# schmrlng/MotionPlanning.jl

Measured on AMD Instinct MI355X. Metric: edges checked/sec + r-disc queries/sec, FMT* N=1e6 R^6, 1/2/4/8 MI355X, higher is better.
Workload: dtype f64

## Files before the change

motionplanning.jl_amd/csrc/kernels_order.hip:

```cpp
#include "mpfmt_internal.h"
#include <algorithm>

#define ORD_ID(k) ((k) & 0x03ffffffu)
#define ORD_COL(k) (((k) >> 26) & 15u)
#define ORD_THREADS 512
#define ORD_WAVES 8
#define ORD_COLS 16
#define ORD_NB 128
#define ORD_STG 2560
#define ORD_PRE 5
#define ORD_WAVES_EU 8
static_assert(ORD_STG >= MPFMT_ORD_MAXDEG, "a column the host lets through must fit the staging area");
static_assert(ORD_COLS * ORD_NB == ORD_THREADS * 4, "the segmented scan gives every thread four buckets");
static_assert(ORD_PRE * ORD_THREADS >= ORD_STG && ORD_STG % 32 == 0 && ORD_STG < 65536, "the prefetched records cover what the staging area holds; positions fit 16 bits");

struct ord_hdr {
    int32_t k[ORD_COLS];
    int32_t cb[ORD_COLS + 4];
    long long out[ORD_COLS];
    int32_t ho[ORD_COLS];
    int32_t n, pad_[3];
};
struct ord_shared {
    uint32_t cnt[ORD_COLS][ORD_NB / 2];
    uint32_t cur[ORD_COLS][ORD_NB / 2];
    ord_hdr h[2];
    int32_t g1, pcount, nextk, pad_;
    uint32_t bits[ORD_STG / 32];
};

__device__ __forceinline__ void lds_barrier()
{
    asm volatile("s_waitcnt lgkmcnt(0)\n\ts_barrier" ::: "memory");
}

struct ord_args {
    const uint32_t* qkey;
    const double* qd2;
    long long qcap;
    const int32_t* qlen;
    const int64_t* degs;
    int64_t tile_begin, tile_end;
    const int64_t* colptr;
    const int32_t* perm;
    const int32_t* iperm;
    int32_t* rowval;
    double* nzval;
    int32_t* rowpos;
    uint32_t bucket_mul;
    const int32_t* spec_fail;
    unsigned long long* mask;
    const int64_t* nnz_dev;
    uint4* pend_items; int64_t pend_wcap; int32_t* pend_cnt; int32_t* pend_over;
    int64_t* deg_clear;
    int rec_bits;
    int32_t* qctr;
};

__global__ __launch_bounds__(ORD_THREADS) __attribute__((amdgpu_waves_per_eu(ORD_WAVES_EU, ORD_WAVES_EU))) void k_order_logs(ord_args a)
{
    if (a.spec_fail && *a.spec_fail) return;
    extern __shared__ __attribute__((aligned(16))) char ord_smem[];
    double* const stage_d2 = reinterpret_cast<double*>(ord_smem);
    uint32_t* const stage_key = reinterpret_cast<uint32_t*>(ord_smem + ORD_STG * 8);
    ord_shared& sh = *reinterpret_cast<ord_shared*>(ord_smem + ORD_STG * 12);
    const int tid = threadIdx.x, lane = tid & 63;
    const int wave = __builtin_amdgcn_readfirstlane(tid >> 6);
    const int64_t nq = (a.tile_end - a.tile_begin) * 4;
    auto bucket = [&](uint32_t id) -> int { return a.bucket_mul ? min(ORD_NB - 1, (int)__umulhi(id, a.bucket_mul)) : (int)(id & (ORD_NB - 1)); };
    if (a.rec_bits && blockIdx.x == 0 && tid == 0) {
        const int64_t nnz = *a.nnz_dev;
        if (nnz & 63) atomicAnd(&a.mask[nnz >> 6], (1ull << (nnz & 63)) - 1ull);
    }

    int hk = 0, ho = -1, hln = 0;
    long long hout = 0;
    auto hdr_fetch1 = [&](int64_t qi) {
        hk = 0; ho = -1; hln = 0;
        if (qi >= nq) return;
        if (tid < ORD_COLS) {
            const int64_t sp = a.tile_begin * 64 + qi * ORD_COLS + tid;
            ho = a.perm[sp];
            hk = (int)a.degs[sp];
            if (a.deg_clear && ho >= 0) a.deg_clear[ho] = 0;
        } else if (tid == 64) {
            hln = (int)min((long long)a.qlen[qi], a.qcap);
        }
    };
    auto hdr_fetch2 = [&]() { hout = (tid < ORD_COLS && ho >= 0) ? a.colptr[ho] : 0; };
    auto hdr_publish = [&](int hb) {
        ord_hdr& H = sh.h[hb];
        if (tid < 64) {
            const int k = (tid < ORD_COLS && ho >= 0) ? hk : 0;
            int inc = k;
            inc += __builtin_amdgcn_update_dpp(0, inc, 0x111, 0xf, 0xf, true);
            inc += __builtin_amdgcn_update_dpp(0, inc, 0x112, 0xf, 0xf, true);
            inc += __builtin_amdgcn_update_dpp(0, inc, 0x114, 0xf, 0xf, true);
            inc += __builtin_amdgcn_update_dpp(0, inc, 0x118, 0xf, 0xf, true);
            if (tid < ORD_COLS) { H.k[tid] = k; H.cb[tid + 1] = inc; H.ho[tid] = ho; }
            if (tid == 0) H.cb[0] = 0;
        } else if (tid == 64) {
            H.n = hln;
        }
    };
    uint32_t pk[ORD_PRE];
    double pd[ORD_PRE];
    auto rec_fetch_n = [&](int total, int64_t qi) {
        const __amdgpu_buffer_rsrc_t rk = __builtin_amdgcn_make_buffer_rsrc(const_cast<uint32_t*>(a.qkey + (qi < nq ? qi : 0) * a.qcap), 0, total * 4, 0x00020000);
#pragma unroll
        for (int u = 0; u < ORD_PRE; ++u) pk[u] = __builtin_amdgcn_raw_buffer_load_b32(rk, tid * 4, u * ORD_THREADS * 4, 0);
    };
    auto rec_fetch = [&](const ord_hdr& H, int64_t qi) { rec_fetch_n((qi < nq) ? H.n : 0, qi); };
    typedef uint32_t ord_u32x2 __attribute__((ext_vector_type(2)));
    auto d2_fetch = [&](int total, int64_t qi) {
        const long long base = (qi < nq ? qi : 0) * a.qcap;
        const __amdgpu_buffer_rsrc_t rd = __builtin_amdgcn_make_buffer_rsrc(const_cast<double*>(a.qd2 + base), 0, total * 8, 0x00020000);
#pragma unroll
        for (int u = 0; u < ORD_PRE; ++u) {
            const ord_u32x2 v = __builtin_amdgcn_raw_buffer_load_b64(rd, tid * 8, u * ORD_THREADS * 8, 0);
            pd[u] = __hiloint2double((int)v.y, (int)v.x);
        }
    };

    if (tid == 0) sh.pcount = 0;
    int64_t qi = blockIdx.x;
    int64_t qn = qi + gridDim.x;
    const int xcd = (int)(blockIdx.x & 7u);
    int hb = 0;
    hdr_fetch1(qi);
    hdr_fetch2();
    hdr_publish(0);
    if (tid < ORD_COLS) sh.h[0].out[tid] = hout;
    lds_barrier();
    rec_fetch(sh.h[0], qi);
    d2_fetch(sh.h[0].n, qi);
    for (; qi < nq; hb ^= 1) {
        const ord_hdr& H = sh.h[hb];
        const int total = H.n;
        const long long lbase = qi * a.qcap;
        hdr_fetch1(qn);
            int g0 = 0;
        bool first = true;
        while (g0 < ORD_COLS) {
            if (tid < 64) {
                const bool ok = tid >= g0 && tid < ORD_COLS && (H.cb[min(tid, ORD_COLS - 1) + 1] - H.cb[g0] <= ORD_STG);
                const unsigned long long m = __ballot(ok);
                if (tid == 0) sh.g1 = g0 + (int)__popcll(m);
            }
            *reinterpret_cast<uint2*>(&sh.cnt[0][tid * 2]) = make_uint2(0u, 0u);
            lds_barrier();
            int g1 = sh.g1;
            const bool skip = g1 == g0;
            if (skip) g1 = g0 + 1;
            const int gb = H.cb[g0];
            auto for_records = [&](auto&& f) {
                if (first) {
#pragma unroll
                    for (int u = 0; u < ORD_PRE; ++u) if (u * ORD_THREADS + tid < total) {
                        uint32_t key = pk[u];
                        asm volatile("" : "+v"(key));
                        f(key, u, u * ORD_THREADS + tid);
                    }
                }
                for (int i = (first ? ORD_PRE * ORD_THREADS : 0) + tid; i < total; i += ORD_THREADS) f(a.qkey[lbase + i], -1, i);
            };
            if (!skip) for_records([&](uint32_t key, int, int) {
                const int col = (int)ORD_COL(key);
                if (col >= g0 && col < g1) { const int bk = bucket(ORD_ID(key)); atomicAdd(&sh.cnt[col][bk >> 1], 1u << ((bk & 1) * 16)); }
            });
            lds_barrier();
            {
                const int col = tid >> 5;
                const uint2 cw = *reinterpret_cast<const uint2*>(&sh.cnt[0][tid * 2]);
                const int c0 = (int)(cw.x & 0xffffu), c1 = (int)(cw.x >> 16), c2 = (int)(cw.y & 0xffffu), c3 = (int)(cw.y >> 16);
                const int tot = c0 + c1 + c2 + c3;
                int inc = tot;
                inc += __builtin_amdgcn_update_dpp(0, inc, 0x111, 0xf, 0xf, true);
                inc += __builtin_amdgcn_update_dpp(0, inc, 0x112, 0xf, 0xf, true);
                inc += __builtin_amdgcn_update_dpp(0, inc, 0x114, 0xf, 0xf, true);
                inc += __builtin_amdgcn_update_dpp(0, inc, 0x118, 0xf, 0xf, true);
                inc += __builtin_amdgcn_update_dpp(0, inc, 0x142, 0xa, 0xf, false);
                const int b0 = min(max(H.cb[col] - gb + inc - tot, 0), ORD_STG);
                const int b1 = min(b0 + c0, ORD_STG), b2 = min(b1 + c1, ORD_STG), b3 = min(b2 + c2, ORD_STG);
                *reinterpret_cast<uint2*>(&sh.cur[0][tid * 2]) = make_uint2((uint32_t)b0 | ((uint32_t)b1 << 16), (uint32_t)b2 | ((uint32_t)b3 << 16));
            }
            lds_barrier();
            if (!skip) for_records([&](uint32_t key, int u, int i) {
                const int col = (int)ORD_COL(key);
                if (col >= g0 && col < g1) {
                    const int bk = bucket(ORD_ID(key));
                    const int pos = (int)((atomicAdd(&sh.cur[col][bk >> 1], 1u << ((bk & 1) * 16)) >> ((bk & 1) * 16)) & 0xffffu);
                    double d2 = 0.0;
                    if (u < 0) d2 = a.qd2[lbase + i];
#pragma unroll
                    for (int v = 0; v < ORD_PRE; ++v) if (u == v) d2 = pd[v];
                    if (pos >= 0 && pos < ORD_STG) { stage_key[pos] = key; stage_d2[pos] = d2; }
                }
            });
            if (a.rec_bits && tid < ORD_STG / 32) sh.bits[tid] = 0xffffffffu;
            lds_barrier();
            if (first) {
                hdr_fetch2();
                hdr_publish(hb ^ 1);
                if (a.qctr && tid == 0) sh.nextk = atomicAdd(&a.qctr[xcd], 1);
                first = false;
            }
            const bool last_range = g1 >= ORD_COLS;
            if (last_range) {
                lds_barrier();
                rec_fetch(sh.h[hb ^ 1], qn);
                d2_fetch(qn < nq ? sh.h[hb ^ 1].n : 0, qn);
            }
            if (!skip) {
                const int nst = min(H.cb[g1] - gb, ORD_STG);
                for (int p0 = 0; p0 < nst; p0 += ORD_THREADS) {
                    const int p = p0 + tid;
                    const bool act = p < nst;
                    if (p0 + wave * 64 >= nst) break;
                    const uint32_t key = act ? stage_key[p] : ((uint32_t)(g1 - 1) << 26);
                    const int col = (int)ORD_COL(key);
                    const uint32_t id = ORD_ID(key);
                    const int bk = bucket(id);
                    const int e = (int)((sh.cur[col][bk >> 1] >> ((bk & 1) * 16)) & 0xffffu), n = (int)((sh.cnt[col][bk >> 1] >> ((bk & 1) * 16)) & 0xffffu);
                    int rk = e - n;
                    if (act) {
                        const int b0 = e - n, bl = e - 1;
                        const uint32_t m0 = ORD_ID(stage_key[b0]), m1 = ORD_ID(stage_key[min(b0 + 1, bl)]), m2 = ORD_ID(stage_key[min(b0 + 2, bl)]),
                                       m3 = ORD_ID(stage_key[min(b0 + 3, bl)]);
                        rk += (int)(m0 < id) + (int)(n > 1 && m1 < id) + (int)(n > 2 && m2 < id) + (int)(n > 3 && m3 < id);
                        for (int m = b0 + 4; m < e; ++m) rk += (ORD_ID(stage_key[m]) < id) ? 1 : 0;
                    }
                    const int rel = rk - (H.cb[col] - gb);
                    const bool valid = act && rel >= 0 && rel < H.k[col];
                    const int64_t o = H.out[col] + rel;
                    int32_t rp = 0;
                    const bool pd_ = valid && a.pend_items && ((key >> 30) & 1u);
                    if ((valid && a.rowpos) || pd_) rp = a.iperm[id];
                    if (valid) {
                        a.rowval[o] = (int32_t)id;
                        a.nzval[o] = sqrt(stage_d2[p]);
                        if (a.rowpos) a.rowpos[o] = rp;
                    }
                    if (a.rec_bits && valid && (key >> 31)) atomicAnd(&sh.bits[rk >> 5], ~(1u << (rk & 31)));
                    if (a.pend_items) {
                        const unsigned long long pm = __ballot(pd_);
                        if (pm) {
                            int base = 0;
                            if (lane == 0) base = atomicAdd(&sh.pcount, (int)__popcll(pm));
                            base = __builtin_amdgcn_readfirstlane(base);
                            if (pd_) {
                                const int pos = base + (int)__builtin_amdgcn_mbcnt_hi((uint32_t)(pm >> 32), __builtin_amdgcn_mbcnt_lo((uint32_t)pm, 0u));
                                if (pos < a.pend_wcap)
                                    a.pend_items[(int64_t)blockIdx.x * a.pend_wcap + pos] =
                                        make_uint4((uint32_t)(uint64_t)o, (uint32_t)((uint64_t)o >> 32), (uint32_t)H.ho[col], (uint32_t)rp);
                            }
                        }
                    }
                }
            }
            lds_barrier();
            if (a.rec_bits) {
                if (!skip) for (int c = g0 + 2 * wave; c < min(g1, g0 + 2 * wave + 2); ++c) {
                    const int k = H.k[c];
                    if (k == 0) continue;
                    const int sb = H.cb[c] - gb;
                    const int64_t o = H.out[c];
                    const int64_t w0 = o >> 6;
                    const int nw = (int)(((o + k - 1) >> 6) - w0) + 1;
                    for (int i = lane; i < nw; i += 64) {
                        const int64_t wd = w0 + i;
                        const int64_t lo_bit = max(wd * 64, o), hi_bit = min(wd * 64 + 64, o + k);
                        const int nb = (int)(hi_bit - lo_bit);
                        const int src = sb + (int)(lo_bit - o);
                        const int wi = src >> 5, sh5 = src & 31;
                        const unsigned long long a0 = sh.bits[wi], a1 = sh.bits[min(wi + 1, ORD_STG / 32 - 1)], a2 = sh.bits[min(wi + 2, ORD_STG / 32 - 1)];
                        unsigned long long val = (a0 | (a1 << 32)) >> sh5;
                        if (sh5) val |= a2 << (64 - sh5);
                        const unsigned long long keep = (nb == 64) ? ~0ull : ((1ull << nb) - 1ull);
                        const int dsh = (int)(lo_bit & 63);
                        const unsigned long long rng = keep << dsh;
                        const unsigned long long w64 = ((val & keep) << dsh) | ~rng;
                        if (w64 != ~0ull) atomicAnd(&a.mask[wd], w64);
                    }
                }
                lds_barrier();
            }
            g0 = g1;
        }
        if (tid < ORD_COLS) sh.h[hb ^ 1].out[tid] = hout;
        qi = qn;
        qn = a.qctr ? 2 * (int64_t)gridDim.x + xcd + 8 * (int64_t)sh.nextk : qn + gridDim.x;
    }
    if (a.pend_items) {
        lds_barrier();
        if (tid == 0) {
            const int c = sh.pcount;
            a.pend_cnt[blockIdx.x] = (int32_t)min((int64_t)c, a.pend_wcap);
            if (c > a.pend_wcap) *a.pend_over = 1;
        }
    }
}

int32_t mpfmt_mask_preset(mpfmt_ctx* ctx, int64_t entries)
{
    int32_t rc;
    const int64_t words = (entries + 63) / 64;
    if ((rc = ctx->graph_free.ensure(ctx, sizeof(uint64_t) * (size_t)(words + 1)))) return rc;
    HIPCHK(ctx, hipMemsetAsync(ctx->graph_free, 0xFF, sizeof(uint64_t) * (size_t)std::max<int64_t>(words, 1), ctx->stream));
    ctx->mask_preset_words = words;
    return MPFMT_OK;
}

int32_t mpfmt_order_logs(mpfmt_ctx* ctx, const int32_t* spec_fail, int64_t mask_entries)
{
    const int64_t nt = ctx->tile_end - ctx->tile_begin;
    int32_t rc;
    ctx->rowpos_valid = false;
    const bool recbits = ctx->bits_in_records;
    const bool pend = ctx->broad_in_drain && !recbits;
    if (recbits) {
        const int64_t words = (std::max<int64_t>(ctx->nnz, mask_entries) + 63) / 64;
        const int64_t words_alloc = (std::max<int64_t>((int64_t)((double)ctx->nnz * 1.02) + 4096, mask_entries) + 63) / 64 + 1;
        if ((rc = ctx->graph_free.ensure(ctx, sizeof(uint64_t) * (size_t)words_alloc))) return rc;
        if (!(ctx->mask_preset_words == words && ctx->nnz > 0))
            HIPCHK(ctx, hipMemsetAsync(ctx->graph_free, ctx->nnz > 0 ? 0xFF : 0, sizeof(uint64_t) * (size_t)std::max<int64_t>(words, 1), ctx->stream));
    }
    ctx->mask_preset_words = -1;
    if (ctx->nnz == 0 || nt <= 0) { if ((rc = mpfmt_side_join(ctx))) return rc; if (recbits) { ctx->graph_swept = true; ctx->sweep_epoch += 1; ctx->sweep_in_order = true; } return MPFMT_OK; }
    const bool want_rowpos = !pend && !recbits;
    if (want_rowpos && (rc = ctx->rowpos.ensure(ctx, sizeof(int32_t) * (size_t)std::max<int64_t>(std::max(ctx->nnz, ctx->nnz_cap), 1)))) return rc;
    const size_t lds = (size_t)ORD_STG * 12 + sizeof(ord_shared);
    HIPCHK(ctx, hipFuncSetAttribute((const void*)k_order_logs, hipFuncAttributeMaxDynamicSharedMemorySize, (int)lds));
    if (ctx->ord_per_cu == 0) {
        int per_cu = 0;
        HIPCHK(ctx, hipOccupancyMaxActiveBlocksPerMultiprocessor(&per_cu, k_order_logs, ORD_THREADS, lds));
        ctx->ord_per_cu = std::max(1, std::min(per_cu, 4));
    }
    unsigned nb = (unsigned)std::min<int64_t>(nt * 4, (int64_t)ctx->num_cus * ctx->ord_per_cu);
    const bool draw = ctx->ord_draw && ctx->ord_ctr && nb >= 8 && (ctx->ord_draw > 1 || ctx->nnz >= (int64_t)1536 * nt * 4);
    if (draw) nb &= ~3u;
    if (pend) {
        const int64_t entries = std::max<int64_t>(ctx->nnz, ctx->nnz_cap);
        ctx->pend_wcap = ctx->debug_small_lists ? 8 : entries * 3 / (2 * (int64_t)nb) + 4096;
        if ((rc = ctx->pend_items.ensure(ctx, sizeof(uint4) * (size_t)ctx->pend_wcap * nb))) return rc;
        if ((rc = ctx->pend_cnt.ensure(ctx, sizeof(int32_t) * (size_t)(nb + 1)))) return rc;
        ctx->pend_over = ctx->pend_cnt + nb;
        HIPCHK(ctx, hipMemsetAsync(ctx->pend_over, 0, sizeof(int32_t), ctx->stream));
    }
    ord_args a{};
    a.qkey = ctx->qkey; a.qd2 = ctx->qd2; a.qcap = ctx->qcap; a.qlen = ctx->qlen; a.degs = ctx->degs;
    a.tile_begin = ctx->tile_begin; a.tile_end = ctx->tile_end; a.colptr = ctx->colptr; a.perm = ctx->perm; a.iperm = ctx->iperm;
    a.rowval = ctx->rowval; a.nzval = ctx->nzval; a.rowpos = want_rowpos ? ctx->rowpos : nullptr;
    a.bucket_mul = ctx->N > 128 ? (uint32_t)((128ull << 32) / (uint64_t)ctx->N) : 0u;
    a.spec_fail = spec_fail;
    a.mask = (unsigned long long*)ctx->graph_free.get(); a.nnz_dev = ctx->colptr + ctx->N;
    a.pend_items = pend ? (uint4*)ctx->pend_items.get() : nullptr; a.pend_wcap = ctx->pend_wcap; a.pend_cnt = ctx->pend_cnt; a.pend_over = ctx->pend_over;
    a.rec_bits = recbits ? 1 : 0;
    a.deg_clear = ctx->world > 1 ? ctx->deg : nullptr;
    a.qctr = draw ? ctx->ord_ctr : nullptr;
    if ((rc = mpfmt_side_join(ctx))) return rc;
    hipLaunchKernelGGL(k_order_logs, dim3(nb), dim3(ORD_THREADS), lds, ctx->stream, a);
    HIPCHK(ctx, hipGetLastError());
    if (pend) ctx->pend_nseg = (int)nb;
    ctx->pend_valid = pend;
    ctx->rowpos_valid = want_rowpos;
    if (recbits) { ctx->graph_swept = true; ctx->sweep_epoch += 1; ctx->sweep_in_order = true; }
    return MPFMT_OK;
}
```

motionplanning.jl_amd/csrc/mpfmt_internal.h:

```cpp
#pragma once
#include <hip/hip_runtime.h>
#include <stdint.h>
#include <cmath>
#include <string>
#include <map>
#include <utility>
#include <vector>
#include "../../include/mpfmt.h"
#include "mpfmt_host.h"

#define MPFMT_WAVE 64
#define MPFMT_MAXS 16

struct mpfmt_timer {
    double total_ms = 0.0;
    int64_t launches = 0;
};

struct mpfmt_grid {
    int32_t gd;
    int32_t g[MPFMT_MAX_DIM];
    double  lo[MPFMT_MAX_DIM];
    double  w[MPFMT_MAX_DIM];
    double  inv_w[MPFMT_MAX_DIM];
    int64_t stride[MPFMT_MAX_DIM];
    int32_t split[MPFMT_MAX_DIM];
    int32_t ext[MPFMT_MAX_DIM];
    int64_t hstride[MPFMT_MAX_DIM];
    int32_t nsplit;
    int64_t inner;
    int64_t ncells;
};
__host__ __device__ __forceinline__ int mpfmt_cell_of(double x, double lo, double inv_w, int g)
{
    double f = floor((x - lo) * inv_w);
    int c = (int)f;
    if (!(f >= 0.0)) c = 0;
    if (f >= (double)g) c = g - 1;
    return c;
}
__host__ __device__ __forceinline__ int64_t mpfmt_cell_term(const mpfmt_grid& G, int i, int c)
{
    const int s = G.split[i];
    return (s > 0 && c >= s) ? G.hstride[i] + (int64_t)(c - s) * G.stride[i] : (int64_t)c * G.stride[i];
}
__host__ __device__ __forceinline__ int mpfmt_cell_coord(const mpfmt_grid& G, int i, int64_t id)
{
    const int64_t in = id % G.inner;
    int c = (int)((in / G.stride[i]) % G.ext[i]);
    if (G.split[i] > 0 && ((id / G.hstride[i]) & 1)) c += G.split[i];
    return c;
}

struct mpfmt_boxes_dev {
    const double* lohi;
    int32_t M;
    int32_t dw;
};

struct mpfmt_ss {
    int32_t has;
    int32_t d;
    double lo[MPFMT_MAX_DIM];
    double hi[MPFMT_MAX_DIM];
};

#define MPFMT_MAX_POLY 16
struct mpfmt_shape2d {
    int32_t kind, n;
    double c[2], r;
    double xr[2], yr[2];
    double pts[MPFMT_MAX_POLY][2], normals[MPFMT_MAX_POLY][2], nex[MPFMT_MAX_POLY][2];
};
struct mpfmt_aabb2d { double xr[2], yr[2]; };

struct mpfmt_ctx;
struct mpfmt_wf;
struct mpfmt_comm;
struct mpfmt_timer_state;
int32_t mpfmt_fail(mpfmt_ctx* ctx, int32_t code, const char* fmt, ...);

template <class T, bool PINNED> struct mpfmt_buf {
    mpfmt_buf() = default;
    mpfmt_buf(const mpfmt_buf&) = delete;
    mpfmt_buf& operator=(const mpfmt_buf&) = delete;
    mpfmt_buf(mpfmt_buf&& o) noexcept { swap(o); }
    mpfmt_buf& operator=(mpfmt_buf&& o) noexcept { swap(o); return *this; }
    ~mpfmt_buf() { reset(); }
    void swap(mpfmt_buf& o) noexcept { std::swap(p_, o.p_); std::swap(bytes_, o.bytes_); }
    void reset()
    {
        if (p_) { if (PINNED) hipHostFree(p_); else hipFree(p_); }
        p_ = nullptr; bytes_ = 0;
    }
    int32_t ensure(mpfmt_ctx* ctx, size_t bytes)
    {
        if (bytes == 0) bytes = 16;
        if (p_ && bytes_ >= bytes) return MPFMT_OK;
        reset();
        void* q = nullptr;
        const hipError_t e = PINNED ? hipHostMalloc(&q, bytes, hipHostMallocDefault) : hipMalloc(&q, bytes);
        if (e != hipSuccess)
            return mpfmt_fail(ctx, MPFMT_ERR_HIP, "%s of %zu bytes failed: %s", PINNED ? "hipHostMalloc" : "hipMalloc", bytes, hipGetErrorString(e));
        p_ = (T*)q; bytes_ = bytes;
        return MPFMT_OK;
    }
    operator T*() const { return p_; }
    T* operator->() const { return p_; }
    T* get() const { return p_; }
    size_t bytes() const { return bytes_; }
private:
    T* p_ = nullptr;
    size_t bytes_ = 0;
};
template <class T> using mpfmt_dbuf = mpfmt_buf<T, false>;
template <class T> using mpfmt_hbuf = mpfmt_buf<T, true>;

struct mpfmt_tmp {
    std::vector<void*> p;
    mpfmt_tmp() = default;
    mpfmt_tmp(const mpfmt_tmp&) = delete;
    mpfmt_tmp& operator=(const mpfmt_tmp&) = delete;
    ~mpfmt_tmp() { for (void* q : p) hipFree(q); }
    template <class T> hipError_t get(T** out, size_t bytes)
    {
        void* q = nullptr;
        const hipError_t e = hipMalloc(&q, bytes ? bytes : 16);
        if (e == hipSuccess) { p.push_back(q); *out = (T*)q; }
        return e;
    }
};

enum mpfmt_steer : int32_t { MPFMT_STEER_DI = 1, MPFMT_STEER_DUBINS = 2, MPFMT_STEER_REEDSSHEPP = 3 };

struct mpfmt_ctx {
    int device = 0;
    hipStream_t stream = nullptr;
    hipStream_t own_stream = nullptr;
    hipStream_t side_stream = nullptr;
    hipEvent_t ev_fork = nullptr, ev_join = nullptr;
    bool side_pending = false;
    int64_t preset_entries = -1;
    int64_t mask_preset_words = -1;
    bool masks_early = false;
    int32_t overlap = 1;
    hipStream_t copy_stream[2] = {nullptr, nullptr};
    hipEvent_t ev_conv[2] = {nullptr, nullptr}, ev_copy[2] = {nullptr, nullptr};
    mpfmt_hbuf<void> export_arena;
    std::string err;
    int rank = 0, world = 1;

    int64_t N = 0;
    int32_t d = 0;
    mpfmt_dbuf<double> Xo;
    mpfmt_dbuf<double> Xo_next;
    double bb_lo[MPFMT_MAX_DIM], bb_hi[MPFMT_MAX_DIM];
    mpfmt_dbuf<void> bb_dev;
    mpfmt_hbuf<void> bb_host;

    double grid_r = -1.0;
    mpfmt_grid grid;
    int64_t ntiles = 0;
    mpfmt_dbuf<int32_t> perm;
    mpfmt_dbuf<int32_t> iperm;
    mpfmt_dbuf<uint32_t> cellkey;
    mpfmt_dbuf<void> idx_arena;
    int32_t* cellstart = nullptr;
    int32_t* list_max = nullptr;
    mpfmt_dbuf<int32_t> cellcnt_pad;
    bool list_max_clean = false;
    uint8_t* tileneed = nullptr;
    uint8_t* tileneed_buf = nullptr;
    int32_t index_halo = 1;
    int32_t shard_blocks = 1;
    int index_rank = 0, index_world = 1;
    std::vector<double> cut_frac;
    std::vector<int64_t> cut_key;
    mpfmt_dbuf<double> Xt;
    mpfmt_dbuf<double> tile_lo;
    mpfmt_dbuf<double> tile_hi;
    mpfmt_dbuf<double> tile_sub;
    mpfmt_dbuf<float> tile_sub32;

    double graph_r = -1.0;
    bool graph_counted = false, graph_filled = false;
    int32_t S = 1;
    int64_t tile_begin = 0, tile_end = 0;
    mpfmt_dbuf<int32_t> slice_cnt;
    mpfmt_dbuf<int64_t> deg;
    mpfmt_dbuf<int64_t> degs;
    mpfmt_dbuf<int64_t> tptr;
    bool tptr_valid = false;
    mpfmt_dbuf<double> Xs;
    mpfmt_dbuf<void> ops;
    double mf_scale = 1.0;
    double ops_r = -1.0;
    int32_t rdisc_path = 0;
    int32_t rdisc_path_used = 0;
    bool filter_valu = false;
    int32_t cell_fb_max = 8;
    int64_t mf_tail_min_items = 32768;
    int32_t ord_draw = 1;
    int32_t mf_tail_permille = 80, mf_tail_slices = 9;
    int32_t mf_xcd_mode = -1;
    int32_t num_cus = 256;
    int ord_per_cu = 0;
    mpfmt_dbuf<int> sweep_ctr;
    int32_t sweep_rounds = 1;
    mpfmt_dbuf<int64_t> rt_cnt;
    mpfmt_dbuf<int64_t> rt_off;
    mpfmt_dbuf<void> rt_tmp;
    mpfmt_dbuf<void> rt_table;
    mpfmt_dbuf<int64_t> rt_total;
    mpfmt_dbuf<double> rt_ss;
    mpfmt_ss rt_ss_host;
    bool rt_ss_valid = false;
    int64_t samples_epoch = 0, ssflag_epoch = -1;
    mpfmt_ss ssflag_ss;
    bool ssflag_all_in = false;
    mpfmt_dbuf<int32_t> ssflag_dev;
    int64_t mf_target_items = 40000;
    float mf_negT = 0.f;
    mpfmt_dbuf<void> lists;
    mpfmt_dbuf<int32_t> list_len;
    mpfmt_dbuf<void> lists_stage;
    int64_t list_cap = 0;
    double lists_r = -1.0; int64_t lists_begin = -1, lists_end = -1;
    int32_t use_pool = 1;
    int64_t qcap = 0;
    mpfmt_dbuf<uint32_t> qkey;
    mpfmt_dbuf<double> qd2;
    const double* st_C = nullptr; const uint64_t* st_H = nullptr; int st_free = 0;
    mpfmt_dbuf<void> st_best; mpfmt_dbuf<int32_t> st_besti, st_nfree;
    mpfmt_dbuf<void> smask;
    int64_t pool_hint_qmax = 0;
    int use_half = 1;
    int fuse_broad = 2;
    mpfmt_dbuf<void> pend_items;
    int64_t pend_wcap = 0;
    mpfmt_dbuf<int32_t> pend_cnt;
    int32_t* pend_over = nullptr;
    int pend_nseg = 0;
    bool sweep_pending_used = false;
    bool pend_overflowed = false;
    bool pend_valid = false;
    mpfmt_dbuf<void> pair_items;
    int64_t pair_icap = 0;
    int pair_slack = 1;
    bool sweep_in_order = false;
    bool bits_in_records = false;
    int debug_small_lists = 0;
    bool want_broad = false;
    bool broad_in_drain = false;
    bool half_used = false;
    int64_t redo_count = 0; int32_t redo_reason = 0;
    bool pool_skip_once = false;
    bool lists_half = false;
    int cell_fb = 0;
    int64_t max_deg = 0;
    int32_t pool_slack = 1;
    bool pool_valid = false;
    bool spec_ready = false;
    bool spec_lists = false;
    bool cnt_pool = false, cnt_mf = false;
    mpfmt_dbuf<int32_t> spec_fail;
    int64_t nnz_cap = 0;
    mpfmt_dbuf<void> rb_dev;
    mpfmt_hbuf<void> rb_host;
    int64_t lists_cap_trusted = -1;
    int64_t pool_hint_N = -1; double pool_hint_r = -1.0; int64_t pool_hint_nnz = 0; int64_t pool_hint_maxdeg = 0; int pool_hint_rank = -1, pool_hint_world = -1;
    int64_t survivors = 0;
    mpfmt_dbuf<int64_t> colptr;
    int64_t nnz = 0;
    mpfmt_dbuf<int32_t> rowtmp;
    mpfmt_dbuf<double> valtmp;
    mpfmt_dbuf<int32_t> rowval;
    mpfmt_dbuf<double> nzval;
    mpfmt_dbuf<int32_t> rowpos;
    bool rowpos_valid = false;
    mpfmt_dbuf<uint64_t> graph_free;
    bool graph_swept = false;
    bool deg_zero_valid = false;
    mpfmt_dbuf<void> zarena;
    mpfmt_dbuf<unsigned long long> d_pairs_own;
    mpfmt_dbuf<int32_t> pool_flag_own, pair_cnt_own, qlen_own;
    unsigned long long* d_pairs = nullptr;
    int32_t* pool_flag = nullptr;
    int32_t* pair_cnt = nullptr;
    int32_t* pair_over = nullptr;
    int32_t* qlen = nullptr;
    int32_t* ord_ctr = nullptr;
    int64_t pairs_tested = 0;

    int64_t knn_k = 0;
    mpfmt_dbuf<uint64_t> knn_mutual;
    mpfmt_dbuf<double> knn_st;
    mpfmt_dbuf<void> knn_bitmap;
    mpfmt_dbuf<void> knn_lists;
    int64_t knn_pairs = 0, knn_rounds = 0, knn_short = 0, knn_scan = 0;

    mpfmt_steer steer_kind = MPFMT_STEER_DI;
    double steer_r = 0.0;
    bool steer_counted = false, steer_filled = false, steer_swept = false;
    mpfmt_dbuf<uint8_t> steer_nseg;
    int32_t di_S = 1;
    double di_rho = 1.0;
    mpfmt_dbuf<int32_t> di_pool_i; mpfmt_dbuf<double> di_pool_c, di_pool_t;
    int64_t di_pool_cap = 0; bool di_pool_valid = false;
    mpfmt_dbuf<void> di_ops;
    bool di_mf = false; float di_negT = 0.f;
    int32_t di_path = 0;
    double car_rt = 1.0, car_sp = 1.0;
    mpfmt_dbuf<uint64_t> car_keep;
    mpfmt_ctx* aux = nullptr;
    mpfmt_dbuf<double> tvaltmp;
    mpfmt_dbuf<double> tval;

    mpfmt_dbuf<double> boxes;
    std::vector<double> boxes_host;
    int32_t M = 0, dw = 0;
    bool have_boxes = false;
    int32_t cc_kind = 0;
    mpfmt_dbuf<mpfmt_shape2d> shapes2d;
    mpfmt_aabb2d aabb2d;
    mpfmt_ss ss;
    mpfmt_dbuf<int32_t> bd_cols;
    mpfmt_dbuf<unsigned long long> bd_ctr;
    int32_t bd_path = 0;
    int64_t bd_columns = 0, bd_entries = 0;

    mpfmt_dbuf<void> scratch;
    std::map<std::string, mpfmt_timer> timers;
    mpfmt_timer_state* timer_state = nullptr;
    bool timing_enabled = true;
    bool rebuild_index = false;

    mpfmt_comm* comm = nullptr;
    int32_t step_state = 0; double step_r = 0.0;
    int32_t wf_graphs = 0;
    int32_t wf_pos_space = 1;
    int64_t wf_seen_epoch = -1; double wf_seen_r = -1.0; int64_t wf_seen_nnz = -1;
    int32_t wf_pos_used = 0;
    int32_t wf_force_sharded = 0;
    mpfmt_wf* wf = nullptr;

    mpfmt_dbuf<double> sssp_C;
    mpfmt_dbuf<int64_t> sssp_A;
    mpfmt_dbuf<uint64_t> sssp_bm;
    mpfmt_dbuf<void> sssp_state;
    mpfmt_hbuf<void> sssp_state_host;
    mpfmt_dbuf<uint64_t> sssp_F;
    hipEvent_t sssp_ev[2] = {nullptr, nullptr};
    int64_t sssp_rounds = 0, sssp_relax = 0, sssp_reached = 0;
    mpfmt_dbuf<unsigned long long> sssp_to_best;
    mpfmt_dbuf<int64_t> sssp_to_tgt;
    mpfmt_dbuf<void> sssp_to_state;
    mpfmt_hbuf<void> sssp_to_state_host;
    int64_t sssp_to_atomics = 0, sssp_to_entries = 0, sssp_to_columns = 0;

    int64_t shortcut_tests = 0, shortcut_checks = 0;
    int64_t disc_steps = 0, disc_samples = 0;

    mpfmt_dbuf<double> sssp_seed;
    int64_t roadmap_candidates = 0, roadmap_near_total = 0;
    int64_t steer_roadmap_steered = 0;

    mpfmt_dbuf<double> ms_L;
    mpfmt_dbuf<int64_t> ms_A;
    mpfmt_dbuf<uint64_t> ms_bm;
    mpfmt_dbuf<void> ms_state;
    mpfmt_hbuf<void> ms_state_host;
    mpfmt_dbuf<void> ms_stage;
    mpfmt_dbuf<int64_t> ms_src;
    hipEvent_t ms_ev[2] = {nullptr, nullptr};
    int64_t ms_groups = 0, ms_rounds = 0, ms_rows = 0, ms_bytes = 0;

    int64_t graph_epoch = 0, sweep_epoch = 0;
    bool graph_imported = false;
    mpfmt_dbuf<double> fld_C;
    mpfmt_dbuf<int64_t> fld_A;
    mpfmt_dbuf<int64_t> fld_Ab;
    mpfmt_dbuf<uint64_t> fld_bm;
    mpfmt_dbuf<void> fld_state;
    mpfmt_hbuf<void> fld_state_host;
    bool fld_tracked = false;
    int64_t fld_source0 = -1; int32_t fld_checkpts = 0;
    int64_t fld_samples_epoch = -1, fld_graph_epoch = -1, fld_sweep_epoch = -1, fld_N = 0, fld_knn_k = 0;
    double fld_graph_r = -1.0;
    bool fld_dirty_any = false;
    int32_t fld_path = 0;
    int64_t fld_invalidated = 0, fld_dirty_columns = 0, fld_columns_read = 0, fld_column_visits = 0, fld_entries_read = 0, fld_rounds = 0,
            fld_relax = 0, fld_reached = 0;

    int64_t steer_epoch = 0, steer_sweep_epoch = 0;
    mpfmt_dbuf<double> tg_G;
    mpfmt_dbuf<unsigned long long> tg_S;
    mpfmt_dbuf<unsigned long long> tg_best;
    mpfmt_dbuf<uint64_t> tg_bm;
    mpfmt_dbuf<int64_t> tg_tgt;
    mpfmt_dbuf<void> tg_state;
    mpfmt_hbuf<void> tg_state_host;
    std::vector<int64_t> tg_targets;
    bool tg_tracked = false, tg_steer = false;
    int32_t tg_checkpts = 0;
    int64_t tg_samples_epoch = -1, tg_build_epoch = -1, tg_sweep_epoch = -1, tg_N = 0, tg_knn_k = 0;
    double tg_graph_r = -1.0, tg_steer_a = 0.0, tg_steer_b = 0.0;
    mpfmt_steer tg_steer_kind = MPFMT_STEER_DI;
    bool tg_dirty_any = false;
    int32_t tg_path = 0, tg_seed_form = 0;
    int64_t tg_invalidated = 0, tg_dirty_columns = 0, tg_columns_read = 0, tg_column_visits = 0, tg_entries_read = 0, tg_rounds = 0,
            tg_relax = 0, tg_atomics = 0, tg_reached = 0;
};

#define HIPCHK(ctx, call)                                                                          \
    do {                                                                                           \
        hipError_t e_ = (call);                                                                    \
        if (e_ != hipSuccess)                                                                      \
            return mpfmt_fail((ctx), MPFMT_ERR_HIP, "%s failed: %s (%s:%d)", #call,                \
                              hipGetErrorString(e_), __FILE__, __LINE__);                          \
    } while (0)

int32_t mpfmt_scratch(mpfmt_ctx* ctx, size_t bytes, void** out);
inline int32_t mpfmt_own_pairs(mpfmt_ctx* ctx)
{
    if (ctx->d_pairs) return MPFMT_OK;
    const int32_t rc = ctx->d_pairs_own.ensure(ctx, 514 * sizeof(unsigned long long));
    ctx->d_pairs = ctx->d_pairs_own;
    return rc;
}
inline int32_t mpfmt_own_pool_flag(mpfmt_ctx* ctx)
{
    if (ctx->pool_flag) return MPFMT_OK;
    const int32_t rc = ctx->pool_flag_own.ensure(ctx, sizeof(int32_t));
    ctx->pool_flag = ctx->pool_flag_own;
    return rc;
}
int32_t mpfmt_states_host(mpfmt_ctx* ctx, int k, std::vector<double>& X, std::vector<double>& P);
void mpfmt_time_begin(mpfmt_ctx* ctx);
void mpfmt_time_end(mpfmt_ctx* ctx, const char* name);
void mpfmt_time_abandon(mpfmt_ctx* ctx);
struct mpfmt_timed {
    mpfmt_ctx* ctx; bool open;
    explicit mpfmt_timed(mpfmt_ctx* c) : ctx(c), open(true) { mpfmt_time_begin(c); }
    void end(const char* name) { if (open) { mpfmt_time_end(ctx, name); open = false; } }
    ~mpfmt_timed() { if (open) mpfmt_time_abandon(ctx); }
    mpfmt_timed(const mpfmt_timed&) = delete;
    mpfmt_timed& operator=(const mpfmt_timed&) = delete;
};

int32_t mpfmt_side_fork(mpfmt_ctx* ctx, hipStream_t* main_out);
int32_t mpfmt_side_back(mpfmt_ctx* ctx, hipStream_t main);
int32_t mpfmt_side_join(mpfmt_ctx* ctx);

int32_t mpfmt_build_grid(mpfmt_ctx* ctx, double r, bool whole = false);
int32_t mpfmt_launch_rdisc_count(mpfmt_ctx* ctx, double r);
int32_t mpfmt_rdisc_count_launch(mpfmt_ctx* ctx, double r, bool spec);
int32_t mpfmt_rdisc_count_finish(mpfmt_ctx* ctx, double r, bool* spec_failed);
int32_t mpfmt_graph_step(mpfmt_ctx* ctx, double r);
int32_t mpfmt_graph_step_launch_impl(mpfmt_ctx* ctx, double r);
int32_t mpfmt_graph_step_finish_impl(mpfmt_ctx* ctx);
int32_t mpfmt_launch_rdisc_fill(mpfmt_ctx* ctx, double r);
int32_t mpfmt_mfma_prepare(mpfmt_ctx* ctx, double r, float* negT_out, bool* usable);
int32_t mpfmt_mfma_build_operands(mpfmt_ctx* ctx);
template <int MODE> int32_t mpfmt_launch_rdisc_mfma(mpfmt_ctx* ctx, double r, float negT);
int32_t mpfmt_order_logs(mpfmt_ctx* ctx, const int32_t* spec_fail = nullptr, int64_t mask_entries = -1);
int32_t mpfmt_mask_preset(mpfmt_ctx* ctx, int64_t entries);
int32_t mpfmt_sweep_prepare_ss(mpfmt_ctx* ctx);
#define MPFMT_ORD_MAXDEG 2048
int32_t mpfmt_mfma_build_lists(mpfmt_ctx* ctx, double r, bool* usable, bool spec = false, bool half = false);
int mpfmt_slices_for(const mpfmt_ctx* ctx, int64_t units, bool mfma);
int32_t mpfmt_launch_log_degrees(mpfmt_ctx* ctx);
int32_t mpfmt_launch_sample_masks(mpfmt_ctx* ctx, double r, void* zero = nullptr, size_t zero_bytes = 0, bool* zeroed = nullptr);
int32_t mpfmt_rdisc_stream_impl(mpfmt_ctx* ctx, double r, const double* C_host, const uint64_t* H_host, int32_t want_free,
                                int64_t* deg, int64_t* nfree, int64_t* parent, double* cost, int64_t* nnz_out);
int32_t mpfmt_launch_exact_pairs(mpfmt_ctx* ctx, const int32_t* spec_fail);
size_t mpfmt_scan_tmp_bytes(size_t n);
int32_t mpfmt_scan_i64_tmp(mpfmt_ctx* ctx, const int64_t* in, int64_t* out, size_t n, void* tmp);
int32_t mpfmt_scan_i64(mpfmt_ctx* ctx, const int64_t* in, int64_t* out, size_t n);
int32_t mpfmt_launch_rdisc_query(mpfmt_ctx* ctx, int64_t v0, double r, int64_t* k_out,
                                 int64_t* inds_host, double* ds_host, int64_t cap);

int32_t mpfmt_knn_build(mpfmt_ctx* ctx, int64_t k);

int32_t mpfmt_launch_points_free(mpfmt_ctx* ctx, const int64_t* d_idx1, int64_t n, uint64_t* d_mask);
int32_t mpfmt_2d_launch_points(mpfmt_ctx* ctx, const double* X, const int64_t* idx1, int64_t n, uint64_t* d_mask);
int32_t mpfmt_2d_launch_edges(mpfmt_ctx* ctx, const int64_t* s1, const int64_t* t1, const double* P, const double* Q, int64_t E, uint64_t* d_mask);
int32_t mpfmt_2d_launch_graph(mpfmt_ctx* ctx);
int32_t mpfmt_launch_states_free(mpfmt_ctx* ctx, const double* d_P, int64_t n, uint64_t* d_mask);
int32_t mpfmt_launch_edges_free(mpfmt_ctx* ctx, const int64_t* d_src1, const int64_t* d_dst1, int64_t E, uint64_t* d_mask);
int32_t mpfmt_launch_motions_free(mpfmt_ctx* ctx, const double* d_P, const double* d_Q, int64_t n, uint64_t* d_mask);
int32_t mpfmt_launch_mc_edges(mpfmt_ctx* ctx, const int64_t* d_src1, const int64_t* d_dst1, int64_t E, double sigma, int64_t rollouts,
                              uint64_t seed, unsigned long long* d_hits);
int32_t mpfmt_launch_mc_is_edges(mpfmt_ctx* ctx, const int64_t* d_src1, const int64_t* d_dst1, int64_t E, double sigma, int64_t rollouts,
                                 uint64_t seed, unsigned long long* d_wsum);
int32_t mpfmt_launch_mc_ais_edges(mpfmt_ctx* ctx, const int64_t* d_src1, const int64_t* d_dst1, int64_t E, double sigma, int64_t rollouts,
                                  uint64_t seed, unsigned long long* d_wsum, double* d_mu);
int32_t mpfmt_launch_graph_sweep(mpfmt_ctx* ctx, const int32_t* spec_fail = nullptr, int64_t mask_entries = -1);

int32_t mpfmt_boxdelta_apply(mpfmt_ctx* ctx, const double* d_delta, int32_t nd, bool remove);
int32_t mpfmt_di_delta_launch(mpfmt_ctx* ctx, const double* d_delta, int32_t nd, bool remove);
int32_t mpfmt_car_delta_launch(mpfmt_ctx* ctx, const double* d_delta, int32_t nd, bool remove);
bool mpfmt_di_sweep_fits(int64_t M, int m);

#include <functional>
#include <vector>
int32_t mpfmt_csc_transpose_device(mpfmt_ctx* ctx, mpfmt_csr_host* out);
int32_t mpfmt_csc_transpose_resident(mpfmt_ctx* ctx, int64_t* d_rowptr, int32_t* d_colidx);
int32_t mpfmt_car_build(mpfmt_ctx* ctx, mpfmt_steer kind, double rt, double sp, double r);
int32_t mpfmt_car_sweep(mpfmt_ctx* ctx);
int32_t mpfmt_car_steer_batch(mpfmt_ctx* ctx, mpfmt_steer kind, const double* d_X0, const double* d_X1, int64_t n, double rt, double sp, double* d_cost,
                              double* d_ctrl, int32_t* d_nseg);
struct di_args;
int32_t mpfmt_di_mf_prepare(mpfmt_ctx* ctx, double rho, double r, float* negT, bool* usable, double* sp_out, double* sv_out, double* pc);
int32_t mpfmt_di_mf_build_operands(mpfmt_ctx* ctx, double sp, double sv, const double* pc_host);
int32_t mpfmt_di_mf_launch(mpfmt_ctx* ctx, const di_args& a, int mode, float negT, unsigned nblk);
int32_t mpfmt_di_count(mpfmt_ctx* ctx, double rho, double r);
int32_t mpfmt_di_fill(mpfmt_ctx* ctx);
int32_t mpfmt_di_sweep(mpfmt_ctx* ctx);
int32_t mpfmt_di_steer_launch(mpfmt_ctx* ctx, int m, const double* dX0, const double* dX1, int64_t n, double rho, double r,
                              double* dcost, double* dt);

int32_t mpfmt_comm_allgather_inplace(mpfmt_ctx* ctx, void* buf, size_t bytes_per_rank, hipStream_t stream);
int32_t mpfmt_comm_world(const mpfmt_ctx* ctx, int* rank, int* world);

int32_t mpfmt_launch_euclid_steer(mpfmt_ctx* ctx, const int64_t* d_src1, const int64_t* d_dst1, int64_t E, double* d_t, double* d_u);
int32_t mpfmt_launch_euclid_propagate(mpfmt_ctx* ctx, const int64_t* d_src1, int64_t E, const double* d_t, const double* d_u,
                                      const double* d_s, double* d_out);

void mpfmt_wf_free(mpfmt_ctx* ctx);
int32_t mpfmt_wf_run(mpfmt_ctx* ctx);
int32_t mpfmt_wf_begin_directed(mpfmt_ctx* ctx, int64_t init_idx, int32_t checkpts, const uint64_t* F_host, int32_t goal_kind,
                                const double* goal_params, int32_t gd, double band, int32_t flags);
void mpfmt_wf_info_now(mpfmt_ctx* ctx, mpfmt_wf_info* info);

int32_t mpfmt_sssp_device(mpfmt_ctx* ctx, int64_t source0, const uint64_t* d_F, double* C_host, int64_t* A_host, mpfmt_sssp_info* info);
void mpfmt_sssp_free(mpfmt_ctx* ctx);
void mpfmt_sssp_to_launch_successors(mpfmt_ctx* ctx, const uint64_t* d_F, const double* G, const uint64_t* bm, unsigned long long* best,
                                     unsigned long long* S);
int32_t mpfmt_sssp_to_device(mpfmt_ctx* ctx, const int64_t* targets1, int64_t ntgt, const uint64_t* d_F, double* G_host, int64_t* S_host,
                             mpfmt_sssp_info* info);
int32_t mpfmt_field_compute(mpfmt_ctx* ctx, int64_t source0, int32_t checkpts, const uint64_t* d_F, mpfmt_field_info* info);
int32_t mpfmt_field_repair(mpfmt_ctx* ctx, const uint64_t* d_F, mpfmt_field_info* info);
int32_t mpfmt_dirty_columns_into(mpfmt_ctx* ctx, unsigned long long* D);
int32_t mpfmt_field_mark_dirty(mpfmt_ctx* ctx);
void mpfmt_field_drop_internal(mpfmt_ctx* ctx);
bool mpfmt_field_live(mpfmt_ctx* ctx);
bool mpfmt_field_history(const mpfmt_ctx* ctx);
int32_t mpfmt_togo_compute(mpfmt_ctx* ctx, const int64_t* targets1, int64_t ntgt, int32_t checkpts, const uint64_t* d_F, mpfmt_togo_info* info);
int32_t mpfmt_togo_repair(mpfmt_ctx* ctx, const uint64_t* d_F, mpfmt_togo_info* info);
int32_t mpfmt_togo_mark_dirty(mpfmt_ctx* ctx);
void mpfmt_togo_drop_internal(mpfmt_ctx* ctx);
bool mpfmt_togo_live(mpfmt_ctx* ctx);
bool mpfmt_togo_history(const mpfmt_ctx* ctx);
int32_t mpfmt_sssp_seeded_device(mpfmt_ctx* ctx, const int64_t* d_idx1, const double* d_dist, const uint8_t* d_bits, int64_t n, const uint64_t* d_F,
                                 mpfmt_sssp_info* info);

struct mpfmt_rm_list {
    int64_t* ptr = nullptr; int64_t* idx1 = nullptr; double* dist = nullptr; uint8_t* bits = nullptr;
    std::vector<int64_t> ptr_host, usable_host;
    int64_t total = 0;
};
int32_t mpfmt_roadmap_grid(mpfmt_ctx* ctx);
int32_t mpfmt_roadmap_lists(mpfmt_ctx* ctx, mpfmt_tmp& tmp, const double* d_Q, int64_t nq, int dir, const uint64_t* d_F, mpfmt_rm_list* out,
                            bool count_only = false);
int32_t mpfmt_roadmap_reduce(mpfmt_ctx* ctx, mpfmt_tmp& tmp, const double* d_Q, int64_t nq, const double* d_C, double* d_cost, int64_t* d_parent);
int32_t mpfmt_roadmap_goal(mpfmt_ctx* ctx, const mpfmt_rm_list& L, int64_t q, const double* d_C, const int64_t* d_A, int64_t* d_res);
int32_t mpfmt_steer_roadmap_lists(mpfmt_ctx* ctx, mpfmt_tmp& tmp, const double* d_Q, int64_t nq, int dir, const uint64_t* d_F, mpfmt_rm_list* out,
                                  bool count_only, const double* d_X, int64_t nx, bool pair);
int32_t mpfmt_steer_roadmap_reduce(mpfmt_ctx* ctx, mpfmt_tmp& tmp, const double* d_Q, int64_t nq, const double* d_C, double* d_cost, int64_t* d_parent);

int32_t mpfmt_sssp_multi_device(mpfmt_ctx* ctx, const int64_t* sources1, int64_t nsrc, const uint64_t* d_F, double* C_host, int64_t* A_host,
                                mpfmt_sssp_info* info);
int32_t mpfmt_roadmap_matrix_device(mpfmt_ctx* ctx, const double* d_S, int64_t ns, const double* d_G, int64_t ng, const uint64_t* d_F,
                                    const uint64_t* d_sfree, const uint64_t* d_gfree, const uint64_t* d_direct, const mpfmt_rm_list& Ls,
                                    const mpfmt_rm_list& Lg, double* d_cost, int32_t* d_status, mpfmt_roadmap_matrix_info* info);
int32_t mpfmt_roadmap_pairs(mpfmt_ctx* ctx, const double* d_S, int64_t ns, const double* d_G, int64_t ng, double* d_P, double* d_Q);
void mpfmt_sssp_multi_free(mpfmt_ctx* ctx);

int32_t mpfmt_shortcut_batch_device(mpfmt_ctx* ctx, const double* P, const int64_t* offsets, int64_t B, int32_t iterations, int64_t max_states,
                                    double* out_P, int64_t* out_offsets, int64_t out_cap, double* cumcost, mpfmt_shortcut_info* info);

int32_t mpfmt_discretize_batch_device(mpfmt_ctx* ctx, int32_t space, int32_t d, const double* params, const double* P, const int64_t* offsets,
                                      int64_t B, int32_t mode, double dt, int64_t n_samples, int32_t append_end, double* out_X, double* out_T,
                                      int32_t* out_seg, int64_t* out_offsets, int64_t out_cap, mpfmt_disc_info* info);

int32_t mpfmt_launch_expand(mpfmt_ctx* ctx, const uint64_t* d_W, const uint64_t* d_H, const uint64_t* d_F,
                            const double* d_C, const int64_t* d_zs1, int64_t nz,
                            int64_t* d_xs, int64_t* d_ymin, double* d_cmin, uint8_t* d_free, int64_t cap,
                            int64_t* nx_host);
```

Measured before the change: 31.01 billion.

## Specialize order kernel per output form and deepen header/work-draw pipeline

The order kernel is templated on its output form (rowpos, pending items, or record bits), so each launch compiles only its own path and drops the runtime branches and iperm loads it does not need. Header fetching is restructured so wave 0 loads perm, degs and qlen, and the colptr loads, publish and work-counter draw are moved earlier, with the queue index now prefetched two steps ahead. Key and d2 prefetches are merged with scalarized bases and sched barriers. The grid is rounded to a multiple of 8 when drawing work, and occupancy is cached per form. In exchange there is more template code, and clamping out-of-range headers with sched barriers could constrain scheduling.

```diff
diff --git a/motionplanning.jl_amd/csrc/kernels_order.hip b/motionplanning.jl_amd/csrc/kernels_order.hip
--- a/motionplanning.jl_amd/csrc/kernels_order.hip
+++ b/motionplanning.jl_amd/csrc/kernels_order.hip
@@ -53,10 +53,10 @@
     const int64_t* nnz_dev;
     uint4* pend_items; int64_t pend_wcap; int32_t* pend_cnt; int32_t* pend_over;
     int64_t* deg_clear;
-    int rec_bits;
     int32_t* qctr;
 };
 
+template <int FORM>
 __global__ __launch_bounds__(ORD_THREADS) __attribute__((amdgpu_waves_per_eu(ORD_WAVES_EU, ORD_WAVES_EU))) void k_order_logs(ord_args a)
 {
     if (a.spec_fail && *a.spec_fail) return;
@@ -68,56 +68,66 @@
     const int wave = __builtin_amdgcn_readfirstlane(tid >> 6);
     const int64_t nq = (a.tile_end - a.tile_begin) * 4;
     auto bucket = [&](uint32_t id) -> int { return a.bucket_mul ? min(ORD_NB - 1, (int)__umulhi(id, a.bucket_mul)) : (int)(id & (ORD_NB - 1)); };
-    if (a.rec_bits && blockIdx.x == 0 && tid == 0) {
+    if constexpr (FORM == 2) if (blockIdx.x == 0 && tid == 0) {
         const int64_t nnz = *a.nnz_dev;
         if (nnz & 63) atomicAnd(&a.mask[nnz >> 6], (1ull << (nnz & 63)) - 1ull);
     }
 
     int hk = 0, ho = -1, hln = 0;
     long long hout = 0;
-    auto hdr_fetch1 = [&](int64_t qi) {
-        hk = 0; ho = -1; hln = 0;
-        if (qi >= nq) return;
-        if (tid < ORD_COLS) {
-            const int64_t sp = a.tile_begin * 64 + qi * ORD_COLS + tid;
-            ho = a.perm[sp];
-            hk = (int)a.degs[sp];
-            if (a.deg_clear && ho >= 0) a.deg_clear[ho] = 0;
-        } else if (tid == 64) {
-            hln = (int)min((long long)a.qlen[qi], a.qcap);
-        }
-    };
-    auto hdr_fetch2 = [&]() { hout = (tid < ORD_COLS && ho >= 0) ? a.colptr[ho] : 0; };
-    auto hdr_publish = [&](int hb) {
+    auto hdr_fetch1 = [&](int64_t q) {
+        if (wave == 0) {
+            const int64_t qc = q < nq ? q : nq - 1;
+            const int64_t sp = a.tile_begin * 64 + qc * ORD_COLS;
+            uint32_t t = (uint32_t)min(tid, ORD_COLS - 1);
+            asm volatile("" : "+v"(t));
+            ho = (a.perm + sp)[t];
+            hk = (int)(a.degs + sp)[t];
+            hln = a.qlen[qc];
+        }
+    };
+    auto hdr_fetch2 = [&](int64_t q) {
+        asm volatile("" : "+v"(ho));
+        const bool own = tid < ORD_COLS && q < nq && ho >= 0;
+        hout = own ? a.colptr[ho] : 0;
+        if (a.deg_clear && own) a.deg_clear[ho] = 0;
+    };
+    auto hdr_publish = [&](int hb, int64_t q) {
         ord_hdr& H = sh.h[hb];
+        asm volatile("" : "+v"(hk), "+v"(hln));
         if (tid < 64) {
-            const int k = (tid < ORD_COLS && ho >= 0) ? hk : 0;
+            const int k = (tid < ORD_COLS && q < nq && ho >= 0) ? hk : 0;
             int inc = k;
             inc += __builtin_amdgcn_update_dpp(0, inc, 0x111, 0xf, 0xf, true);
             inc += __builtin_amdgcn_update_dpp(0, inc, 0x112, 0xf, 0xf, true);
             inc += __builtin_amdgcn_update_dpp(0, inc, 0x114, 0xf, 0xf, true);
             inc += __builtin_amdgcn_update_dpp(0, inc, 0x118, 0xf, 0xf, true);
-            if (tid < ORD_COLS) { H.k[tid] = k; H.cb[tid + 1] = inc; H.ho[tid] = ho; }
-            if (tid == 0) H.cb[0] = 0;
-        } else if (tid == 64) {
-            H.n = hln;
+            if (tid < ORD_COLS) { H.k[tid] = k; H.cb[tid + 1] = inc; H.ho[tid] = q < nq ? ho : -1; }
+            if (tid == 0) { H.cb[0] = 0; H.n = q < nq ? (int)min((long long)hln, a.qcap) : 0; }
         }
     };
     uint32_t pk[ORD_PRE];
     double pd[ORD_PRE];
-    auto rec_fetch_n = [&](int total, int64_t qi) {
-        const __amdgpu_buffer_rsrc_t rk = __builtin_amdgcn_make_buffer_rsrc(const_cast<uint32_t*>(a.qkey + (qi < nq ? qi : 0) * a.qcap), 0, total * 4, 0x00020000);
+    auto uni64 = [](long long v) -> long long {
+        const uint32_t lo = (uint32_t)__builtin_amdgcn_readfirstlane((int)(uint32_t)v), hi = (uint32_t)__builtin_amdgcn_readfirstlane((int)(uint32_t)((unsigned long long)v >> 32));
+        return (long long)(((unsigned long long)hi << 32) | lo);
+    };
+    typedef uint32_t ord_u32x2 __attribute__((ext_vector_type(2)));
+    auto rec_fetch = [&](const ord_hdr& H, int64_t q) {
+        const int total = (q < nq) ? __builtin_amdgcn_readfirstlane(H.n) : 0;
+        const long long base = uni64((q < nq ? q : 0) * a.qcap);
+        const __amdgpu_buffer_rsrc_t rk = __builtin_amdgcn_make_buffer_rsrc(const_cast<uint32_t*>(a.qkey + base), 0, total * 4, 0x00020000);
+        const __amdgpu_buffer_rsrc_t rd = __builtin_amdgcn_make_buffer_rsrc(const_cast<double*>(a.qd2 + base), 0, total * 8, 0x00020000);
+        __builtin_amdgcn_sched_barrier(0);
 #pragma unroll
-        for (int u = 0; u < ORD_PRE; ++u) pk[u] = __builtin_amdgcn_raw_buffer_load_b32(rk, tid * 4, u * ORD_THREADS * 4, 0);
-    };
-    auto rec_fetch = [&](const ord_hdr& H, int64_t qi) { rec_fetch_n((qi < nq) ? H.n : 0, qi); };
-    typedef uint32_t ord_u32x2 __attribute__((ext_vector_type(2)));
-    auto d2_fetch = [&](int total, int64_t qi) {
-        const long long base = (qi < nq ? qi : 0) * a.qcap;
-        const __amdgpu_buffer_rsrc_t rd = __builtin_amdgcn_make_buffer_rsrc(const_cast<double*>(a.qd2 + base), 0, total * 8, 0x00020000);
+        for (int u = 0; u < ORD_PRE; ++u) {
+            pk[u] = __builtin_amdgcn_raw_buffer_load_b32(rk, tid * 4, u * ORD_THREADS * 4, 0);
+            __builtin_amdgcn_sched_barrier(0);
+        }
 #pragma unroll
         for (int u = 0; u < ORD_PRE; ++u) {
             const ord_u32x2 v = __builtin_amdgcn_raw_buffer_load_b64(rd, tid * 8, u * ORD_THREADS * 8, 0);
+            __builtin_amdgcn_sched_barrier(0);
             pd[u] = __hiloint2double((int)v.y, (int)v.x);
         }
     };
@@ -125,21 +135,29 @@
     if (tid == 0) sh.pcount = 0;
     int64_t qi = blockIdx.x;
     int64_t qn = qi + gridDim.x;
+    int64_t q2 = qn + gridDim.x;
     const int xcd = (int)(blockIdx.x & 7u);
     int hb = 0;
+    int drawn = 0;
     hdr_fetch1(qi);
-    hdr_fetch2();
-    hdr_publish(0);
-    if (tid < ORD_COLS) sh.h[0].out[tid] = hout;
+    hdr_publish(0, qi);
+    hdr_fetch2(qi);
+    auto draw = [&]() {
+        if (a.qctr && tid == 0) {
+            int slot = xcd;
+            asm volatile("" : "+v"(slot));
+            drawn = atomicAdd(&a.qctr[slot], 1);
+        }
+    };
+    draw();
     lds_barrier();
     rec_fetch(sh.h[0], qi);
-    d2_fetch(sh.h[0].n, qi);
     for (; qi < nq; hb ^= 1) {
         const ord_hdr& H = sh.h[hb];
-        const int total = H.n;
+        const int total = __builtin_amdgcn_readfirstlane(H.n);
         const long long lbase = qi * a.qcap;
         hdr_fetch1(qn);
-            int g0 = 0;
+        int g0 = 0;
         bool first = true;
         while (g0 < ORD_COLS) {
             if (tid < 64) {
@@ -197,19 +215,22 @@
                     if (pos >= 0 && pos < ORD_STG) { stage_key[pos] = key; stage_d2[pos] = d2; }
                 }
             });
-            if (a.rec_bits && tid < ORD_STG / 32) sh.bits[tid] = 0xffffffffu;
-            lds_barrier();
+            if constexpr (FORM == 2) if (tid < ORD_STG / 32) sh.bits[tid] = 0xffffffffu;
             if (first) {
-                hdr_fetch2();
-                hdr_publish(hb ^ 1);
-                if (a.qctr && tid == 0) sh.nextk = atomicAdd(&a.qctr[xcd], 1);
+                if (tid < ORD_COLS) sh.h[hb].out[tid] = hout;
+                if (a.qctr && tid == 0) sh.nextk = drawn;
+            }
+            lds_barrier();
+            hdr_publish(hb ^ 1, qn);
+            hdr_fetch2(qn);
+            if (first) {
+                draw();
                 first = false;
             }
             const bool last_range = g1 >= ORD_COLS;
             if (last_range) {
                 lds_barrier();
                 rec_fetch(sh.h[hb ^ 1], qn);
-                d2_fetch(qn < nq ? sh.h[hb ^ 1].n : 0, qn);
             }
             if (!skip) {
                 const int nst = min(H.cb[g1] - gb, ORD_STG);
@@ -233,16 +254,16 @@
                     const int rel = rk - (H.cb[col] - gb);
                     const bool valid = act && rel >= 0 && rel < H.k[col];
                     const int64_t o = H.out[col] + rel;
-                    int32_t rp = 0;
-                    const bool pd_ = valid && a.pend_items && ((key >> 30) & 1u);
-                    if ((valid && a.rowpos) || pd_) rp = a.iperm[id];
                     if (valid) {
+                        int32_t rp = 0;
+                        if constexpr (FORM == 0) rp = a.iperm[id];
                         a.rowval[o] = (int32_t)id;
                         a.nzval[o] = sqrt(stage_d2[p]);
-                        if (a.rowpos) a.rowpos[o] = rp;
-                    }
-                    if (a.rec_bits && valid && (key >> 31)) atomicAnd(&sh.bits[rk >> 5], ~(1u << (rk & 31)));
-                    if (a.pend_items) {
+                        if constexpr (FORM == 0) a.rowpos[o] = rp;
+                    }
+                    if constexpr (FORM == 2) if (valid && (key >> 31)) atomicAnd(&sh.bits[rk >> 5], ~(1u << (rk & 31)));
+                    if constexpr (FORM == 1) {
+                        const bool pd_ = valid && ((key >> 30) & 1u);
                         const unsigned long long pm = __ballot(pd_);
                         if (pm) {
                             int base = 0;
@@ -250,16 +271,18 @@
                             base = __builtin_amdgcn_readfirstlane(base);
                             if (pd_) {
                                 const int pos = base + (int)__builtin_amdgcn_mbcnt_hi((uint32_t)(pm >> 32), __builtin_amdgcn_mbcnt_lo((uint32_t)pm, 0u));
-                                if (pos < a.pend_wcap)
+                                if (pos < a.pend_wcap) {
+                                    const int32_t rp = a.iperm[id];
                                     a.pend_items[(int64_t)blockIdx.x * a.pend_wcap + pos] =
                                         make_uint4((uint32_t)(uint64_t)o, (uint32_t)((uint64_t)o >> 32), (uint32_t)H.ho[col], (uint32_t)rp);
+                                }
                             }
                         }
                     }
                 }
             }
             lds_barrier();
-            if (a.rec_bits) {
+            if constexpr (FORM == 2) {
                 if (!skip) for (int c = g0 + 2 * wave; c < min(g1, g0 + 2 * wave + 2); ++c) {
                     const int k = H.k[c];
                     if (k == 0) continue;
@@ -287,11 +310,11 @@
             }
             g0 = g1;
         }
-        if (tid < ORD_COLS) sh.h[hb ^ 1].out[tid] = hout;
         qi = qn;
-        qn = a.qctr ? 2 * (int64_t)gridDim.x + xcd + 8 * (int64_t)sh.nextk : qn + gridDim.x;
-    }
-    if (a.pend_items) {
+        qn = q2;
+        q2 = a.qctr ? 3 * (int64_t)gridDim.x + xcd + 8 * (int64_t)__builtin_amdgcn_readfirstlane(sh.nextk) : q2 + gridDim.x;
+    }
+    if constexpr (FORM == 1) {
         lds_barrier();
         if (tid == 0) {
             const int c = sh.pcount;
@@ -330,15 +353,18 @@
     const bool want_rowpos = !pend && !recbits;
     if (want_rowpos && (rc = ctx->rowpos.ensure(ctx, sizeof(int32_t) * (size_t)std::max<int64_t>(std::max(ctx->nnz, ctx->nnz_cap), 1)))) return rc;
     const size_t lds = (size_t)ORD_STG * 12 + sizeof(ord_shared);
-    HIPCHK(ctx, hipFuncSetAttribute((const void*)k_order_logs, hipFuncAttributeMaxDynamicSharedMemorySize, (int)lds));
-    if (ctx->ord_per_cu == 0) {
+    const int form = recbits ? 2 : (pend ? 1 : 0);
+    void (*const kern)(ord_args) = form == 2 ? k_order_logs<2> : (form == 1 ? k_order_logs<1> : k_order_logs<0>);
+    HIPCHK(ctx, hipFuncSetAttribute((const void*)kern, hipFuncAttributeMaxDynamicSharedMemorySize, (int)lds));
+    if (ctx->ord_per_cu_form[form] == 0) {
         int per_cu = 0;
-        HIPCHK(ctx, hipOccupancyMaxActiveBlocksPerMultiprocessor(&per_cu, k_order_logs, ORD_THREADS, lds));
-        ctx->ord_per_cu = std::max(1, std::min(per_cu, 4));
-    }
+        HIPCHK(ctx, hipOccupancyMaxActiveBlocksPerMultiprocessor(&per_cu, kern, ORD_THREADS, lds));
+        ctx->ord_per_cu_form[form] = std::max(1, std::min(per_cu, 4));
+    }
+    ctx->ord_per_cu = ctx->ord_per_cu_form[form];
     unsigned nb = (unsigned)std::min<int64_t>(nt * 4, (int64_t)ctx->num_cus * ctx->ord_per_cu);
     const bool draw = ctx->ord_draw && ctx->ord_ctr && nb >= 8 && (ctx->ord_draw > 1 || ctx->nnz >= (int64_t)1536 * nt * 4);
-    if (draw) nb &= ~3u;
+    if (draw) nb &= ~7u;
     if (pend) {
         const int64_t entries = std::max<int64_t>(ctx->nnz, ctx->nnz_cap);
         ctx->pend_wcap = ctx->debug_small_lists ? 8 : entries * 3 / (2 * (int64_t)nb) + 4096;
@@ -355,11 +381,10 @@
     a.spec_fail = spec_fail;
     a.mask = (unsigned long long*)ctx->graph_free.get(); a.nnz_dev = ctx->colptr + ctx->N;
     a.pend_items = pend ? (uint4*)ctx->pend_items.get() : nullptr; a.pend_wcap = ctx->pend_wcap; a.pend_cnt = ctx->pend_cnt; a.pend_over = ctx->pend_over;
-    a.rec_bits = recbits ? 1 : 0;
     a.deg_clear = ctx->world > 1 ? ctx->deg : nullptr;
     a.qctr = draw ? ctx->ord_ctr : nullptr;
     if ((rc = mpfmt_side_join(ctx))) return rc;
-    hipLaunchKernelGGL(k_order_logs, dim3(nb), dim3(ORD_THREADS), lds, ctx->stream, a);
+    hipLaunchKernelGGL(kern, dim3(nb), dim3(ORD_THREADS), lds, ctx->stream, a);
     HIPCHK(ctx, hipGetLastError());
     if (pend) ctx->pend_nseg = (int)nb;
     ctx->pend_valid = pend;
diff --git a/motionplanning.jl_amd/csrc/mpfmt_internal.h b/motionplanning.jl_amd/csrc/mpfmt_internal.h
--- a/motionplanning.jl_amd/csrc/mpfmt_internal.h
+++ b/motionplanning.jl_amd/csrc/mpfmt_internal.h
@@ -205,6 +205,7 @@
     int32_t mf_xcd_mode = -1;
     int32_t num_cus = 256;
     int ord_per_cu = 0;
+    int ord_per_cu_form[3] = {0, 0, 0};
     mpfmt_dbuf<int> sweep_ctr;
     int32_t sweep_rounds = 1;
     mpfmt_dbuf<int64_t> rt_cnt;
```

Measured after the change: 30.79 billion. Within noise of the previous version (-0.7%).
